# nannau/DoWnGAN

Measured on AMD Instinct MI355X. Metric: train-step samples/sec (G+D+GP), higher is better.
Workload: dtype bf16

## Files before the change

downgan_amd/_lib.py:

```python
from __future__ import annotations

import ctypes as C
import os

_HERE = os.path.dirname(os.path.abspath(__file__))
LIB_PATH = os.environ.get("DG_LIB_OVERRIDE") or os.path.join(_HERE, "csrc", "libdowngan_hip.so")

DG_F32, DG_BF16 = 0, 1
STATUS = {0: "DG_OK", -1: "DG_ERR_BAD_SHAPE", -2: "DG_ERR_BAD_DTYPE", -3: "DG_ERR_BAD_ARG", -4: "DG_ERR_LAUNCH"}


class Epilogue(C.Structure):
    _fields_ = [("bias", C.c_void_p), ("has_act", C.c_int), ("act_slope", C.c_float),
                ("r1", C.c_void_p), ("ldr1", C.c_int64), ("s1", C.c_float),
                ("r2", C.c_void_p), ("ldr2", C.c_int64), ("s2", C.c_float),
                ("mask", C.c_void_p), ("ldmask", C.c_int64), ("mask_slope", C.c_float),
                ("accumulate", C.c_int), ("mask_bits", C.c_void_p), ("out_bits", C.c_void_p),
                ("mask_c0", C.c_int), ("mask_last", C.c_int), ("out_q", C.c_void_p), ("out_qs", C.c_void_p), ("ldqs", C.c_int64),
                ("out_u", C.c_void_p), ("out_ue", C.c_void_p), ("skip_y", C.c_int), ("out_amax", C.c_void_p)]


class ConvGeom(C.Structure):
    _fields_ = [("dtype", C.c_int), ("N", C.c_int), ("H", C.c_int), ("W", C.c_int),
                ("Cin", C.c_int), ("Cout", C.c_int), ("stride", C.c_int), ("cin_real", C.c_int), ("pixel_shuffle", C.c_int),
# ... 83 lines not shown
class Hist2dAxis(C.Structure):
    _fields_ = [("src", C.c_int), ("chan", C.c_int), ("nbins", C.c_int), ("lo", C.c_float), ("inv_w", C.c_float)]


class Hist2dSpec(C.Structure):
    _fields_ = [("npairs", C.c_int), ("speed_u", C.c_int), ("speed_v", C.c_int), ("nsec", C.c_int), ("calm", C.c_float),
                ("tan_k", C.c_float * (HIST2D_MAX_SECTORS // 4)), ("scale", C.c_float * EOF_MAX_C),
                ("offset", C.c_float * EOF_MAX_C), ("ax", (Hist2dAxis * 2) * HIST2D_MAX_PAIRS)]


class IncrSpec(C.Structure):
    _fields_ = [("speed_u", C.c_int), ("speed_v", C.c_int), ("nlag", C.c_int), ("nbins", C.c_int),
                ("lag", C.c_int * INCR_MAX_LAGS), ("scale", C.c_float * EOF_MAX_C), ("offset", C.c_float * EOF_MAX_C),
                ("lo", (C.c_float * INCR_MAX_LAGS) * HIST_MAX_OUT), ("inv_w", (C.c_float * INCR_MAX_LAGS) * HIST_MAX_OUT)]


class ObjectsSpec(C.Structure):
    _fields_ = [("speed_u", C.c_int), ("speed_v", C.c_int), ("nthr", C.c_int), ("connectivity", C.c_int),
                ("inv_quantum", C.c_float), ("scale", C.c_float * EOF_MAX_C), ("offset", C.c_float * EOF_MAX_C),
                ("thr", (C.c_float * OBJ_MAX_THR) * HIST_MAX_OUT)]


class DistmapSpec(C.Structure):
    _fields_ = [("speed_u", C.c_int), ("speed_v", C.c_int), ("nthr", C.c_int), ("nring", C.c_int), ("cutoff", C.c_int),
                ("scale", C.c_float * EOF_MAX_C), ("offset", C.c_float * EOF_MAX_C),
                ("thr", (C.c_float * DIST_MAX_THR) * HIST_MAX_OUT)]


class TemporalSpec(C.Structure):
    _fields_ = [("speed_u", C.c_int), ("speed_v", C.c_int), ("nthr", C.c_int), ("ndur", C.c_int), ("nlag", C.c_int),
                ("nbins", C.c_int), ("below", C.c_int * TEMPORAL_MAX_THR), ("lag", C.c_int * TEMPORAL_MAX_LAGS),
                ("scale", C.c_float * EOF_MAX_C), ("offset", C.c_float * EOF_MAX_C),
                ("thr", (C.c_float * TEMPORAL_MAX_THR) * HIST_MAX_OUT), ("lo", (C.c_float * TEMPORAL_MAX_LAGS) * HIST_MAX_OUT),
                ("inv_w", (C.c_float * TEMPORAL_MAX_LAGS) * HIST_MAX_OUT)]


MINMAX_PARTS = 256
_vp, _i, _i64, _f = C.c_void_p, C.c_int, C.c_int64, C.c_float
_PROTOS = {
    "dg_conv3x3_fwd": [C.POINTER(ConvGeom), C.POINTER(Epilogue), _vp, _vp, _vp, _vp],
    "dg_conv3x3_dgrad": [C.POINTER(ConvGeom), C.POINTER(Epilogue), _vp, _vp, _vp, _vp],
    "dg_conv3x3_wgrad": [C.POINTER(ConvGeom), _vp, _vp, _vp, _vp, _vp],
    "dg_conv3x3_wgrad_dense": [_vp, _i, _vp, _vp, _vp, _vp, _vp],
    "dg_conv3x3_wgrad_f8": [C.POINTER(ConvGeom), _vp, _vp, _vp, _vp, _vp, _vp],
    "dg_exp_from_amax": [_vp, _i, _i, _vp, _vp],
    "dg_conv3x3_wgrad_dense_f8": [C.POINTER(ConvGeom), _i, _vp, _vp, _vp, _vp, _vp, _vp],
    "dg_gather_gemm": [C.POINTER(GGDesc), C.POINTER(Epilogue), _vp, _vp, _vp, _vp],
    "dg_conv3x3_plan": [C.POINTER(ConvGeom), _i, C.POINTER(GGDesc)],
    "dg_last_conv_kernels": [],
    "dg_last_wgrad_kernel": [],
    "dg_conv3x3_dgrad_launches": [C.POINTER(ConvGeom)],
    "dg_conv3x3_dgrad_stream_eligible": [C.POINTER(ConvGeom), C.POINTER(Epilogue)],
    "dg_set_s2_dgrad_stream": [C.c_int],
    "dg_colsum": [_i, _vp, _i64, _i64, _i64, _i64, _i, _vp, _vp],
    "dg_colsum_multi": [_i, _vp, _i64, _i64, _i, _i, _vp, _vp],
    "dg_repack_conv_weights": [_i, _i, _vp, _vp, _i, _i, _vp],
    "dg_repack_dense_dgrad": [_i, _vp, _i, _i, _vp, _vp],
    "dg_wgrad_unswap": [_vp, _vp, _i, _i, _vp],
    "dg_linear_fwd": [_i, _vp, _i64, _vp, _i64, _vp, _i, _i, _i, _i64, _vp],
    "dg_linear_dx": [_i, _i, _vp, _i, _vp, _i64, _vp, _i64, _vp, _i64, _f, _i, _i, _i64, _vp],
    "dg_linear_dw": [_i, _vp, _i, _vp, _i64, _vp, _i64, _i, _i, _i64, _vp],
    "dg_linear_dw_wide": [_i, _vp, _i, _vp, _i64, _vp, _i64, _i, _i, _i64, _i, _vp],
    "dg_bias_act": [_i, _vp, _i, _vp, _vp, _i, _i, _i, _i, _f, _vp, _i, _f, _vp],
    "dg_mask_mul": [_i, _vp, _i64, _vp, _i64, _i64, _i, _f, _vp],
    "dg_axpby": [_i, _vp, _i64, _vp, _i64, _f, _vp, _i64, _f, _i64, _i, _vp],
    "dg_gp_interp": [_i, _vp, _vp, _vp, _vp, _i, _i64, _vp],
    "dg_gp_interp_c2": [_i, _vp, _vp, _i64, _vp, _vp, _vp, _vp, _i, _i64, _vp],
    "dg_scale_rows_c2": [_i, _vp, _i64, _vp, _vp, _i, _i64, _vp],
    "dg_sumsq_rows": [_i, _vp, _i, _i64, _vp, _vp],
    "dg_gp_finish": [_vp, _i, _i, _f, _f, _vp, _vp, _vp],
    "dg_scale_rows": [_i, _vp, _vp, _vp, _i, _i64, _vp],
    "dg_l1": [_i, _vp, _i64, _vp, _i64, _i64, _i, _vp, _vp, _i64, _f, _vp, _i64, _vp],
    "dg_sqdiff": [_i, _vp, _i64, _vp, _i64, _i64, _i, _vp, _vp],
    "dg_sum_strided": [_vp, _i, _i, _f, _vp, _vp],
    "dg_fill_col": [_vp, _i, _i, _i, _f, _vp],
    "dg_adam": [_vp, _vp, _vp, _vp, _vp, _i64, _f, _f, _f, _f, _i, _f, _vp],
    "dg_nchw_to_nhwc": [_i, _vp, _vp, _i, _i, _i, _i, _i, _vp],
    "dg_nhwc_to_nchw": [_i, _vp, _i64, _vp, _i, _i, _i, _i, _vp],
    "dg_cast": [_i, _vp, _vp, _i64, _vp],
    "dg_minmax_partial": [_i, _vp, _i64, _i64, _i, _vp, _vp],
    "dg_minmax_finish": [_vp, _i, _vp, _vp],
    "dg_normalise_planar": [_i, _vp, _i, _i, _i, _i64, _i, _vp, _vp, _vp],
    "dg_ssim_level": [_vp, _vp, _i, _i, _i, C.POINTER(SsimParams), _vp, _vp],
    "dg_avgpool2": [_vp, _vp, _i, _i, _i, _vp],
    "dg_msssim_finish": [_vp, _i, _i, C.POINTER(MsssimCombine), _vp, _vp],
    "dg_div_vort_sums": [_i, _vp, _i64, _vp, _i64, _i, _i, _i, _vp, _vp],
    "dg_gather_samples": [_i, _vp, _i64, _i, _vp, _i, _vp, _i, _vp],
    "dg_quant_mxfp8": [_i, _vp, _i64, _i64, _i, _vp, _i64, _vp, _i64, _vp],
    "dg_block_exp_max": [_vp, _i64, _i64, _i, _i, _vp, _vp, _vp],
    "dg_block_exp_max_batch": [C.POINTER(ExpBatch), _i, _vp, _vp],
    "dg_quant_uniform": [_i, _vp, _i64, _i64, _i, _vp, _vp, _i64, _vp],
    "dg_conv3x3_fwd_f8": [C.POINTER(ConvGeom), C.POINTER(Epilogue), C.POINTER(F8Operands), _vp, _vp],
    "dg_conv3x3_dgrad_f8": [C.POINTER(ConvGeom), C.POINTER(Epilogue), C.POINTER(F8Operands), _vp, _vp],
    "dg_moments": [_vp, _i64, _vp, _vp],
    "dg_stage_fields": [_i, C.POINTER(FieldPlanes), _i64, _vp, _vp],
    "dg_lowpass5": [_i, _vp, _i64, _i, _i, _i, _i, _vp, _i64, _vp, _i64, _vp],
    "dg_lowpass5_adjoint": [_i, _vp, _i64, _i, _i, _i, _i, _vp, _i64, _vp],
    "dg_set_deterministic_workspace": [_vp, _i64],
    "dg_deterministic": [],
    "dg_count_nonfinite": [C.POINTER(FiniteBufs), _vp, _vp],
    "dg_eof_mean": [C.POINTER(EofFields), _vp, _vp],
    "dg_eof_gram": [C.POINTER(EofFields), _vp, _i, _vp, _vp, _vp],
    "dg_eof_components": [C.POINTER(EofFields), _vp, _vp, _i, _vp, _i64, _i64, _vp, _vp],
    "dg_eof_flip": [_vp, _i, _i, _i, _i64, _i64, _vp, _vp],
    "dg_eof_project": [C.POINTER(EofFields), _vp, _vp, _i, _i64, _i64, _i, _vp, _vp, _vp],
    "dg_eof_reconstruct": [_vp, _i, _i, _i, _vp, _i64, _i64, _i, _vp, _vp, _vp],
# ... 107 lines not shown
```

downgan_amd/engine.py:

```python
from __future__ import annotations

import dataclasses
import math
import os

import torch

from . import layout
from .ops import Conv

G_SLOPE = 0.01
C_SLOPE = 0.2
RES_SCALE = 0.2
FC_HID = 100
FC_HID_P = 112
FC_HID_LD = 128
FC_OUT_P = 16


@dataclasses.dataclass
class HyperParams:
    gp_lambda: float = 10.0
    critic_iterations: int = 5
    batch_size: int = 32
# ... 776 lines not shown
            if f8b:
                o.quant_mxfp8(bw["us"][(3 * i + 2) & 1][..., 4 * F_:], *usq((3 * i + 2) & 1, 4 * F_, 5 * F_))
                if u_live:
                    o.quant_uniform(bw["us"][(3 * i + 2) & 1][..., 4 * F_:], *uu(3 * i + 2, 4 * F_, 5 * F_))
            for j in (2, 1, 0):
                d = 3 * i + j
                slab, us = self._saved[d], bw["us"][d & 1]
                pre = f"res_blocks.{i}.dense_blocks.{j}.b"
                for k in range(4, 0, -1):
                    uk = us[..., (k - 1) * F_:k * F_]
                    kw = dict(xq=usq(d & 1, k * F_, 5 * F_), wq=self._vq[d][k], out_q=usq(d & 1, (k - 1) * F_, k * F_)) if f8b else {}
                    if u_live:
                        kw["out_u"] = uu(d, (k - 1) * F_, k * F_)
                    o.conv_dgrad(self.cv_v[k], us[..., k * F_:], self.vpack(d, k), uk, mask=slab[..., k * F_:(k + 1) * F_], mask_slope=G_SLOPE, **kw)
                if u_live:
                    o.conv_wgrad_dense_f8(self.cv_b, self._slab_u[d], self._ex[d], self._us_u[d & 1], self._eu[d], [GW(f"{pre}{k}.0") for k in range(1, 6)])
                    o.colsum_multi(us, [GB(f"{pre}{k}.0") for k in range(1, 6)])
                else:
                    o.conv_wgrad_dense(self.cv_b, slab, us, [GW(f"{pre}{k}.0") for k in range(1, 6)], [GB(f"{pre}{k}.0") for k in range(1, 6)])
                if self.f8_wg:
                    o.block_exp_max(bw["usq"][d & 1][1], self._eu_new[d])
                nxt = bw["us"][(d - 1) & 1][..., 4 * F_:] if j > 0 else bw["gx"]
                kw = {}
                if f8b:
                    kw = dict(xq=usq(d & 1, 0, 5 * F_), wq=self._vq[d][0])
                    if j > 0:
                        kw["out_q"] = usq((d - 1) & 1, 4 * F_, 5 * F_)
                        if u_live:
                            kw["out_u"] = uu(d - 1, 4 * F_, 5 * F_)
                o.conv_dgrad(self.cv_v[0], us, self.vpack(d, 0), nxt, r1=us[..., 4 * F_:], s1=RES_SCALE, **kw)
            gyn = bw["gy"][gyi ^ 1]
            o.axpby(gyn, bw["gx"], 1.0 / RES_SCALE, gy, 1.0)
            gy, gyi = gyn, gyi ^ 1
        if self.f8_wg and self._ex_new is not None:
            self._ex.copy_(self._ex_new); self._eu.copy_(self._eu_new)
            self._u_ok = True
            self._u_live = False
        o.axpby(gy, gy, 1.0, d_trunk, 1.0)
        o.conv_wgrad(self.cv_conv1, x, gy, GW("conv1"), db=GB("conv1"))


METRIC_SINKS = (("spectra", True), ("coherence", False), ("helmholtz", False), ("distributions", True), ("maps", False),
                ("fss", False), ("joint", False), ("increments", False), ("hist_maps", False), ("temporal", False),
                ("objects", False), ("distances", False))


class TrainEngine:

    SCALARS = ("c_real_mean", "c_fake_mean", "gp_ret", "g_c_fake_mean", "l1_sum")

    def __init__(self, ops, coarse_side, filters, channels, batch, hp: HyperParams = None, n_predictands=2,
                 num_res_blocks=16, num_upsample=3, dist=None, stacked=None, check_finite=False):
        self.ops, self.hp = ops, hp or HyperParams()
        self.check_finite = bool(check_finite)
        self.B, self.S = batch, coarse_side
        self.dist = dist
        self.world = dist.world_size if dist is not None else 1
        fine = coarse_side << num_upsample
        self.G = NativeGenerator(ops, filters, channels, batch, coarse_side, n_predictands, num_res_blocks, num_upsample)
        compact2 = n_predictands <= 2 and fine % 32 == 0 and not any(
            os.environ.get(k) is not None for k in ("DG_NO_COMPACT2", "DG_WG_NOIM2COL", "DG_GG_NOIM2COL"))
        if stacked is None:
            env = os.environ.get("DG_STACKED")
            stacked = (int(env) if env.isdigit() and int(env) > 1 else True) if env is not None else False
        stacked = stacked if (stacked and compact2 and self._fits_stacked(ops, filters, batch, coarse_side, fine, num_res_blocks)) else False
        self.C = NativeCritic(ops, filters, fine, n_predictands, batch, stacked=stacked)
        assert self.C.c_pad[0] == self.G.np_p
        o = ops
        self.fine_shape = (batch, fine, fine, self.G.np_p)
        self.compact2 = compact2 and bool(self.C.convs[0].cin_real)
        self.stacked = self.C.stacked and self.compact2
        cshape = (batch, fine, fine, 2) if self.compact2 else self.fine_shape
        self.gbuf = o.zeros(*self.fine_shape)
        self.vbuf = o.zeros(*cshape)
        if self.compact2:
            self.x3 = o.zeros(3 * batch, fine, fine, 2)
            self.real_c, self.fake_c, self.xhat = self.x3[:batch], self.x3[batch:2 * batch], self.x3[2 * batch:]
        else:
            self.x3 = self.real_c = self.fake_c = None
            self.xhat = o.zeros(*cshape)
        self.dfake = None
        self.ss = o.zeros(batch, dtype=torch.float32)
        self.coef = o.zeros(batch, dtype=torch.float32)
        self.scal = o.zeros(8, dtype=torch.float32)
        self.alpha_dev = o.zeros(batch, dtype=torch.float32)
        self.num_steps = 0
        self.n_real_elems = batch * n_predictands * fine * fine
        self.adam_hp = {}
        self._msssim = {}
        self.graphs = False

    def _sc(self, name):
        i = self.SCALARS.index(name)
        return self.scal[i:i + 1]

    @staticmethod
    def _fits_stacked(ops, filters, batch, coarse_side, fine, nrb):
        if not torch.cuda.is_available() or getattr(ops, "device", None) is None or torch.device(ops.device).type != "cuda":
            return True
        es = 4 if ops.tdtype == torch.float32 else 2
        cd, h, per_c = filters, fine, 0
        for l, st in enumerate(NativeCritic.STRIDES):
            h //= st
            per_c += (cd << (l // 2)) * h * h
        critic = 2 * 3 * batch * per_c * es * 1.07 + 2 * batch * cd * fine * fine * es + 24 * (cd * 8 * (fine // 16) ** 2 * 112 + 5e7 * (cd / 128.0) ** 2)
        S, F_ = coarse_side, filters
# ... 251 lines not shown
```

downgan_amd/ops.py:

```python
from __future__ import annotations

import ctypes as C
import dataclasses

import os
import torch

from . import _lib
from ._lib import ConvGeom, Epilogue, check

TORCH_DTYPE = {"f32": torch.float32, "bf16": torch.bfloat16}
DG_DTYPE = {"f32": _lib.DG_F32, "bf16": _lib.DG_BF16}


@dataclasses.dataclass(frozen=True)
class Conv:
    N: int
    H: int
    W: int
    Cin: int
    Cout: int
    stride: int = 1
    pixel_shuffle: bool = False
    cin_real: int = 0
# ... 16 lines not shown

def pix_layout(t):
    assert t.dim() == 4 and t.stride(3) == 1, (t.shape, t.stride())
    ld = t.stride(2)
    n, h, w, _ = t.shape
    assert (w == 1 or t.stride(2) == ld) and (h == 1 or t.stride(1) == w * ld) and (n == 1 or t.stride(0) == h * w * ld), \
        (t.shape, t.stride())
    return ld, n * h * w


_DET = {"ws": None, "refs": 0}


def _det_acquire(lib, device, nbytes):
    if _DET["ws"] is None or _DET["ws"].numel() < nbytes or _DET["ws"].device != torch.device(device):
        ws = torch.empty(nbytes, dtype=torch.uint8, device=device)
        torch.cuda.synchronize(device)
        check(lib.dg_set_deterministic_workspace(C.c_void_p(ws.data_ptr()), ws.numel()), "dg_set_deterministic_workspace")
        _DET["ws"] = ws
    _DET["refs"] += 1


def _det_release(lib):
    _DET["refs"] = max(0, _DET["refs"] - 1)
    if _DET["refs"] == 0 and _DET["ws"] is not None:
        lib.dg_set_deterministic_workspace(C.c_void_p(0), 0)
        _DET["ws"] = None


class HipOps:

    name = "hip"

    def __init__(self, dtype="bf16", device="cuda:0", f8_critic=False, f8_generator=False, deterministic=None, det_workspace_mb=512):
        assert dtype in TORCH_DTYPE
        if not torch.cuda.is_available():
            raise RuntimeError("downgan_amd.ops.HipOps needs a ROCm GPU (no CPU fallback exists)")
        self.dtype = dtype
        self.tdtype = TORCH_DTYPE[dtype]
        self.dg = DG_DTYPE[dtype]
        self.device = torch.device(device)
        self._dev_index = self.device.index if self.device.index is not None else torch.cuda.current_device()
        self.lib = _lib.lib()
        self.prof = None
        self.f8 = bool(f8_critic or f8_generator)
        self.f8_generator = bool(f8_generator)
        self.f8_wgrad = os.environ.get("DG_NO_F8_WGRAD") is None
        self.f8_gbwd = os.environ.get("DG_NO_F8_GBWD") is None
        self.f8_gwgrad = os.environ.get("DG_NO_F8_GWGRAD") is None
        self.f8_gtail = os.environ.get("DG_NO_F8_GTAIL") is None
        self.f8_l0u = os.environ.get("DG_NO_F8_L0U") is None
        assert not self.f8 or dtype == "bf16", "the fp8 conv path quantises bf16 tensors"
        self._f8_scratch = {}
        if deterministic is None:
            deterministic = os.environ.get("DG_DETERMINISTIC", "0") not in ("", "0")
        self._det_held = False
        if deterministic:
            _det_acquire(self.lib, self.device, int(det_workspace_mb) << 20)
            self._det_held = True
        self._finite_counts = None

    @property
    def deterministic(self):
        return bool(self.lib.dg_deterministic())

    def close(self):
        if self._det_held:
            self._det_held = False
            _det_release(self.lib)

    def __del__(self):
        try:
            self.close()
        except Exception:
            pass

    def count_nonfinite(self, bufs):
        assert 1 <= len(bufs) <= _lib.FINITE_MAX
        f = _lib.FiniteBufs(nbuf=len(bufs))
        for i, (name, t) in enumerate(bufs):
            assert t.is_cuda and t.is_contiguous() and t.dtype in (torch.float32, torch.bfloat16), (name, t.dtype)
            f.ptr[i], f.n[i], f.dtype[i] = t.data_ptr(), t.numel(), (_lib.DG_F32 if t.dtype == torch.float32 else _lib.DG_BF16)
        if self._finite_counts is None:
            self._finite_counts = torch.zeros(_lib.FINITE_MAX, dtype=torch.int32, device=self.device)
        check(self.lib.dg_count_nonfinite(C.byref(f), _ptr(self._finite_counts), self._stream()), "dg_count_nonfinite")
        counts = self._finite_counts.cpu().tolist()
        return {name: int(counts[i]) for i, (name, _) in enumerate(bufs)}

    def _stream(self):
        if torch.cuda.current_device() != self._dev_index:
            torch.cuda.set_device(self.device)
        return C.c_void_p(torch.cuda.current_stream(self.device).cuda_stream)

    per_layer = False

    def _timed(self, tag, flops, fn, nbytes=0.0, net="", geom=""):
        if self.prof is None:
            return fn()
        s, e = torch.cuda.Event(enable_timing=True), torch.cuda.Event(enable_timing=True)
        s.record()
        rc = fn()
        e.record()
        if self.per_layer and geom:
            tag = f"{tag}:{geom}"
        if net:
            tag = f"{tag}:{net}"
# ... 60 lines not shown
        ep.accumulate = int(accumulate)
        for name, t in (("mask_bits", mask_bits), ("out_bits", out_bits)):
            if t is not None:
                assert t.dtype == torch.int16 and t.is_cuda and t.is_contiguous() and tuple(t.shape) == self.bits_shape(out.shape), (name, t.shape, out.shape)
                setattr(ep, name, t.data_ptr())
        assert not (mask is not None and mask_bits is not None)
        if out_q is not None:
            q, qs = out_q
            Cc = out.shape[-1]
            assert out.dtype == torch.bfloat16 and Cc % 64 == 0 and Cc >= 128
            assert q.dtype == torch.uint8 and qs.dtype == torch.uint8 and q.shape == out.shape and q.stride() == out.stride(), (q.shape, q.stride(), out.stride())
            assert tuple(qs.shape) == tuple(out.shape[:-1]) + (Cc // 32,) and qs.stride(-1) == 1
            assert all(qs.stride(i) * out.stride(2) == out.stride(i) * qs.stride(2) for i in range(3)), (qs.stride(), out.stride())
            ep.out_q, ep.out_qs, ep.ldqs = q.data_ptr(), qs.data_ptr(), qs.stride(2)
        if out_u is not None:
            u, ue = out_u
            assert u.dtype == torch.uint8 and u.shape == out.shape and u.stride() == out.stride()
            assert ue.dtype == torch.uint8 and ue.is_contiguous() and ue.numel() == out.shape[-1] // 32
            ep.out_u, ep.out_ue = u.data_ptr(), ue.data_ptr()
        if skip_y:
            assert (out_q is not None or out_u is not None) and not accumulate
            ep.skip_y = 1
        if out_amax is not None:
            assert out_amax.dtype == torch.int32 and out_amax.is_cuda and out_amax.is_contiguous() and out_amax.numel() == out.shape[-1] // 32
            ep.out_amax = out_amax.data_ptr()
        return ep

    def out_shape(self, cv: Conv):
        if cv.pixel_shuffle:
            return (cv.N, 2 * cv.Ho, 2 * cv.Wo, cv.Cout // 4)
        return (cv.N, cv.Ho, cv.Wo, cv.Cout)

    def f8_eligible(self, cv: Conv, kind):
        if kind == "wgrad":
            return (self.f8 and self.f8_wgrad and cv.net == "C" and not cv.pixel_shuffle and cv.Cin % 128 == 0
                    and cv.Cout % 128 == 0 and cv.Wo % 64 == 0)
        cred, nout = (cv.Cin, cv.Cout) if kind == "fwd" else (cv.Cout, cv.Cin)
        nets = ("C", "G") if (self.f8_generator and (kind == "fwd" or self.f8_gbwd)) else ("C",)
        if self.f8_generator and self.f8_gtail and kind == "fwd" and cv.net == "T":
            return cred % 128 == 0 and nout > 64 and (not cv.pixel_shuffle or (cv.Cout // 4) % 32 == 0)
        return self.f8 and cv.net in nets and cred % 128 == 0 and nout > 64 and not cv.pixel_shuffle

    def conv_fwd(self, cv: Conv, x, w_fwd, y, xq=None, wq=None, **ep):
        self._act(x); self._act(y); self._act(w_fwd)
        assert tuple(x.shape) == (cv.N, cv.H, cv.W, cv.Cin) or (cv.cin_real and tuple(x.shape) == (cv.N, cv.H, cv.W, 2) and cv.stride == 1), (x.shape, cv)
        assert tuple(y.shape) == self.out_shape(cv), (y.shape, cv)
        assert w_fwd.numel() == cv.Cout * 9 * cv.Cin and w_fwd.is_contiguous()
        g = self._geom(cv, pix_layout(x)[0], pix_layout(y)[0])
        e = self._epilogue(y, **ep)
        if self.f8_eligible(cv, "fwd"):
            check(self._timed("conv_fwd", self.conv_flops(cv), lambda: self._conv_f8(self.lib.dg_conv3x3_fwd_f8, g, e, x, w_fwd, cv.Cout, cv.Cin, y, xq, wq),
                              self.conv_bytes(cv, ep), cv.net, self._geom_tag(cv)), "dg_conv3x3_fwd_f8")
            return
        check(self._timed("conv_fwd", self.conv_flops(cv), lambda: self.lib.dg_conv3x3_fwd(
            C.byref(g), C.byref(e), _ptr(x), _ptr(w_fwd), _ptr(y), self._stream()), self.conv_bytes(cv, ep), cv.net, self._geom_tag(cv)), "dg_conv3x3_fwd")

    def conv_dgrad(self, cv: Conv, dy, w_dgrad, dx, xq=None, wq=None, **ep):
        self._act(dy); self._act(dx); self._act(w_dgrad)
        assert tuple(dx.shape) == (cv.N, cv.H, cv.W, cv.Cin), (dx.shape, cv)
        assert tuple(dy.shape) == self.out_shape(cv), (dy.shape, cv)
        assert w_dgrad.numel() == cv.Cout * 9 * cv.Cin and w_dgrad.is_contiguous()
        g = self._geom(cv, pix_layout(dx)[0], pix_layout(dy)[0])
        e = self._epilogue(dx, **ep)
        if self.f8_eligible(cv, "dgrad"):
            check(self._timed("conv_dgrad", self.conv_flops(cv), lambda: self._conv_f8(self.lib.dg_conv3x3_dgrad_f8, g, e, dy, w_dgrad, cv.Cin, cv.Cout, dx, xq, wq),
                              self.conv_bytes(cv, ep), cv.net, self._geom_tag(cv)), "dg_conv3x3_dgrad_f8")
            return
        check(self._timed("conv_dgrad", self.conv_flops(cv), lambda: self.lib.dg_conv3x3_dgrad(
            C.byref(g), C.byref(e), _ptr(dy), _ptr(w_dgrad), _ptr(dx), self._stream()), self.conv_bytes(cv, ep), cv.net, self._geom_tag(cv)), "dg_conv3x3_dgrad")

    def quant_mxfp8(self, src, q=None, scales=None):
        Cc = src.shape[-1]
        assert Cc % 128 == 0 and src.stride(-1) == 1 and src.is_cuda and src.dtype in (torch.float32, torch.bfloat16)
        if src.dim() == 4:
            ld, rows = pix_layout(src)
        else:
            assert src.dim() == 2
            ld, rows = src.stride(0), src.shape[0]
        if q is None:
            q = torch.empty(src.shape, dtype=torch.uint8, device=self.device)
            scales = torch.empty(tuple(src.shape[:-1]) + (Cc // 32,), dtype=torch.uint8, device=self.device)
        assert q.dtype == torch.uint8 and scales.dtype == torch.uint8 and q.shape == src.shape and q.stride(-1) == 1 and scales.stride(-1) == 1
        assert tuple(scales.shape) == tuple(src.shape[:-1]) + (Cc // 32,)
        ldq, ldqs = q.stride(-2), scales.stride(-2)
        if src.dim() == 4:
            assert pix_layout(q)[1] == rows and all(scales.stride(i) * ldq == q.stride(i) * ldqs for i in range(3))
        sdt = _lib.DG_F32 if src.dtype == torch.float32 else _lib.DG_BF16
        check(self.lib.dg_quant_mxfp8(sdt, _ptr(src), rows, ld, Cc, _ptr(q), ldq, _ptr(scales), ldqs, self._stream()), "dg_quant_mxfp8")
        return q, scales

    def block_exp_max(self, scales, out, margin=1):
        self.block_exp_max_batch([(scales, out)], margin)

    def block_exp_max_batch(self, pairs, margin=1):
        if self._exp_scratch is None:
            self._exp_scratch = torch.zeros(64 * _lib.EXP_BATCH_MAX, dtype=torch.int32, device=self.device)
        for k in range(0, len(pairs), _lib.EXP_BATCH_MAX):
            b = _lib.ExpBatch()
            chunk = pairs[k:k + _lib.EXP_BATCH_MAX]
            b.n = len(chunk)
            nbytes = 0
            for i, (scales, out) in enumerate(chunk):
                nb = scales.shape[-1]
                assert scales.dtype == torch.uint8 and out.dtype == torch.uint8 and out.numel() == nb and scales.stride(-1) == 1
                assert scales.dim() == 2 or all(scales.stride(d) == scales.stride(d + 1) * scales.shape[d + 1] for d in range(scales.dim() - 2)), scales.stride()
                b.scales[i], b.rows[i], b.ld[i], b.nblocks[i], b.out[i] = scales.data_ptr(), scales.numel() // nb, scales.stride(-2), nb, out.data_ptr()
                nbytes += scales.numel()
# ... 713 lines not shown
```

include/downgan_hip.h:

```cpp
#ifndef DOWNGAN_HIP_H
#define DOWNGAN_HIP_H

#include <stddef.h>
#include <stdint.h>

#ifdef __cplusplus
extern "C" {
#endif

#define DG_F32 0
#define DG_BF16 1

typedef enum dg_status {
  DG_OK = 0,
  DG_ERR_BAD_SHAPE = -1,
  DG_ERR_BAD_DTYPE = -2,
  DG_ERR_BAD_ARG = -3,
  DG_ERR_LAUNCH = -4
} dg_status;

typedef struct dg_epilogue {
  const float* bias;
  int has_act;
  float act_slope;
// ... 27 lines not shown

typedef struct dg_gg_desc {
  int dtype;
  int N, Hs, Ws, Cred; int64_t lds;
  int src_ps;
  int Hg, Wg, sy_mul, sx_mul;
  int ntaps; int tap_dy[9], tap_dx[9], tap_w[9];
  int Nout; int64_t ldw;
  int Hd, Wd; int64_t ldd;
  int dy_mul, dx_mul, dy_off, dx_off;
  int dst_ps;
} dg_gg_desc;

const char* dg_version(void);


int dg_conv3x3_fwd(const dg_conv_geom* g, const dg_epilogue* ep, const void* x, const void* w_fwd,
                   void* y, void* stream);

int dg_conv3x3_dgrad(const dg_conv_geom* g, const dg_epilogue* ep, const void* dy,
                     const void* w_dgrad, void* dx, void* stream);

int dg_conv3x3_wgrad(const dg_conv_geom* g, const void* x, const void* dy, float* dw, float* db,
                     void* stream);

int dg_conv3x3_wgrad_dense(const dg_conv_geom* g, int nconv, const void* x, const void* dy,
                           float* const* dw, float* const* db, void* stream);

int dg_conv3x3_wgrad_f8(const dg_conv_geom* g, const void* xq, const void* ex, const void* dyq, const void* ey, float* dw,
                        void* stream);

int dg_conv3x3_wgrad_dense_f8(const dg_conv_geom* g, int nconv, const void* xq, const void* ex, const void* dyq, const void* ey,
                              float* const* dw, void* stream);

int dg_colsum(int dtype, const void* dy, int64_t rows_outer, int64_t ld_outer, int64_t rows_inner,
              int64_t ld, int C, float* db, void* stream);

int dg_colsum_multi(int dtype, const void* dy, int64_t rows, int64_t ld, int C, int nseg, float* const* db, void* stream);

int dg_gather_gemm(const dg_gg_desc* d, const dg_epilogue* ep, const void* x, const void* w, void* y,
                   void* stream);

int dg_last_conv_kernels(void);

int dg_last_wgrad_kernel(void);

int dg_conv3x3_plan(const dg_conv_geom* g, int kind, dg_gg_desc* out);

int dg_conv3x3_dgrad_launches(const dg_conv_geom* g);

int dg_conv3x3_dgrad_stream_eligible(const dg_conv_geom* g, const dg_epilogue* ep);

int dg_set_s2_dgrad_stream(int on);

int dg_repack_conv_weights(int dtype, int kind, const float* master, void* dst, int CoutP, int CinP,
                           void* stream);
int dg_repack_dense_dgrad(int dtype, const float* const* masters, int nconv, int F, void* dst, void* stream);
int dg_wgrad_unswap(const float* tmp, float* dw, int CoutP, int CinP, void* stream);


int dg_linear_fwd(int dtype, const void* x, int64_t ldx, const void* w, int64_t ldw, float* y,
                  int ldy, int B, int O, int64_t K, void* stream);
int dg_linear_dx(int dtype, int out_dtype, const float* dy, int ldo, const void* w, int64_t ldw,
                 void* dx, int64_t lddx, const void* mask, int64_t ldmask, float mask_slope, int B,
                 int O, int64_t K, void* stream);
int dg_linear_dw(int dtype, const float* dy, int ldo, const void* x, int64_t ldx, float* dw,
                 int64_t lddw, int B, int O, int64_t K, void* stream);
int dg_linear_dw_wide(int dtype, const float* dy, int ldo, const void* x, int64_t ldx, float* dw,
                      int64_t lddw, int B, int O, int64_t K, int accumulate, void* stream);


int dg_bias_act(int out_dtype, const float* in, int ldi, const float* bias, void* out, int ldo,
                int rows, int C, int has_act, float slope, const void* mask, int ldmask,
                float mask_slope, void* stream);
int dg_mask_mul(int dtype, void* u, int64_t ldu, const void* y, int64_t ldy, int64_t rows, int C,
                float slope, void* stream);
int dg_axpby(int dtype, void* out, int64_t ldo, const void* x, int64_t ldx, float a, const void* y,
             int64_t ldy, float b, int64_t rows, int C, void* stream);
int dg_gp_interp(int dtype, const void* real, const void* fake, const float* alpha, void* xhat,
                 int B, int64_t per_img, void* stream);
int dg_gp_interp_c2(int dtype, const void* real, const void* fake, int64_t ld, const float* alpha,
                    void* xhat_c, void* real_c, void* fake_c, int B, int64_t pix_per_img, void* stream);
int dg_scale_rows_c2(int dtype, const void* g, int64_t ld, const float* coef, void* out_c, int B,
                     int64_t pix_per_img, void* stream);
int dg_sumsq_rows(int dtype, const void* g, int B, int64_t per_img, float* ss, void* stream);
int dg_gp_finish(const float* ss, int B, int B_global, float gp_lambda, float weight, float* coef,
                 float* scalars, void* stream);
int dg_scale_rows(int dtype, const void* g, const float* coef, void* out, int B, int64_t per_img,
                  void* stream);
int dg_l1(int dtype, const void* a, int64_t lda, const void* b, int64_t ldb, int64_t rows, int C,
          float* acc, void* grad, int64_t ldg, float grad_scale, const void* addend, int64_t ldadd,
          void* stream);
int dg_sqdiff(int dtype, const void* a, int64_t lda, const void* b, int64_t ldb, int64_t rows, int C,
              float* acc, void* stream);
int dg_sum_strided(const float* in, int n, int stride, float scale, float* out, void* stream);
int dg_fill_col(float* buf, int rows, int ld, int col, float value, void* stream);

int dg_adam(float* p, const float* g, float* m, float* v, void* shadow_bf16, int64_t n, float lr,
            float beta1, float beta2, float eps, int step, float grad_scale, void* stream);

int dg_nchw_to_nhwc(int dtype, const float* src, void* dst, int N, int C, int H, int W, int Cpad,
                    void* stream);
int dg_nhwc_to_nchw(int dtype, const void* src, int64_t lds, float* dst, int N, int C, int H, int W,
                    void* stream);
int dg_cast(int dtype, const float* src, void* dst, int64_t n, void* stream);

// ... 263 lines not shown
```

Baseline: 73.89.

## Add persistent row-streaming 3x3 conv forward kernel with split-K wave handoff

Adds a persistent bf16 3x3 conv forward kernel for Cin=128 stride-1 layers. Each block walks column strips of an image row by row, keeps an 8-row input ring in LDS, and holds weights in registers. Two wave groups each compute half of the input channels and pass partial accumulators through LDS, while the next rows are prefetched with buffer loads. The engine turns this path on by default and falls back to the old kernel for geometries or epilogues it cannot handle. The aim is to cut repeated halo/input loads and launch overhead, at the cost of high register pressure and one block per CU.

```diff
diff --git a/downgan_amd/_lib.py b/downgan_amd/_lib.py
--- a/downgan_amd/_lib.py
+++ b/downgan_amd/_lib.py
@@ -159,6 +159,9 @@
     "dg_conv3x3_dgrad_launches": [C.POINTER(ConvGeom)],
     "dg_conv3x3_dgrad_stream_eligible": [C.POINTER(ConvGeom), C.POINTER(Epilogue)],
     "dg_set_s2_dgrad_stream": [C.c_int],
+    "dg_conv3x3_fwd_stream": [C.POINTER(ConvGeom), C.POINTER(Epilogue), _vp, _vp, _vp, _vp],
+    "dg_conv3x3_fwd_stream_eligible": [C.POINTER(ConvGeom), C.POINTER(Epilogue)],
+    "dg_set_fwd_stream": [C.c_int],
     "dg_colsum": [_i, _vp, _i64, _i64, _i64, _i64, _i, _vp, _vp],
     "dg_colsum_multi": [_i, _vp, _i64, _i64, _i, _i, _vp, _vp],
     "dg_repack_conv_weights": [_i, _i, _vp, _vp, _i, _i, _vp],
diff --git a/downgan_amd/csrc/conv_fwd_stream.hip b/downgan_amd/csrc/conv_fwd_stream.hip
--- /dev/null
+++ b/downgan_amd/csrc/conv_fwd_stream.hip
@@ -0,0 +1,322 @@
+#include "gg_common.h"
+
+namespace {
+
+constexpr int NT = 512;
+constexpr int RING_PIX = 18;
+constexpr int RING_PITCH = 288;
+constexpr int RING_ROW = RING_PIX * RING_PITCH;
+constexpr int RING_SLOTS = 8;
+constexpr int ROW_CHUNKS = RING_PIX * 16;
+constexpr int HAND_OFF = RING_SLOTS * RING_ROW;
+constexpr int HAND_WAVE = 4 * 64 * 16;
+constexpr int HAND_BUF = 4 * HAND_WAVE;
+constexpr int LDS_BYTES = HAND_OFF + 2 * HAND_BUF;
+
+struct FSArgs {
+  const char* x; const char* w; char* y;
+  const float* bias; const char* mask_bits; char* out_bits;
+  float act_slope, mask_slope;
+  int H, W, ldx, ldy;
+  int bpp;
+  int nct;
+  int nstrips, nitems;
+  int nwalk, trips;
+  int xcd_group;
+};
+
+__device__ __forceinline__ __amdgpu_buffer_rsrc_t uniform_rsrc(const char* p) {
+  const unsigned long long b = (unsigned long long)p;
+  const unsigned long long u = ((unsigned long long)(unsigned)__builtin_amdgcn_readfirstlane((int)(unsigned)(b >> 32)) << 32) |
+                               (unsigned)__builtin_amdgcn_readfirstlane((int)(unsigned)b);
+  return __builtin_amdgcn_make_buffer_rsrc((void*)u, 0, (int)DG_OOB_OFF, 0x00020000);
+}
+
+template <int F>
+__device__ __forceinline__ void store_pixel(const FSArgs& a, const f32x4_t& f0, const f32x4_t& f1, unsigned mb, __amdgpu_buffer_rsrc_t rY,
+                                            unsigned off, __amdgpu_buffer_rsrc_t rB, unsigned boff) {
+  float v[8] = {f0[0], f0[1], f0[2], f0[3], f1[0], f1[1], f1[2], f1[3]};
+  if (F & 1) {
+    if (a.act_slope >= 0.f && a.act_slope <= 1.f) {
+      typedef float f32x2_t __attribute__((ext_vector_type(2)));
+      const f32x2_t sl2 = {a.act_slope, a.act_slope};
+#pragma unroll
+      for (int k = 0; k < 8; k += 2) {
+        const f32x2_t p = f32x2_t{v[k], v[k + 1]} * sl2;
+        v[k] = __builtin_fmaxf(v[k], p[0]); v[k + 1] = __builtin_fmaxf(v[k + 1], p[1]);
+      }
+    } else {
+#pragma unroll
+      for (int k = 0; k < 8; ++k) v[k] = leaky(v[k], a.act_slope);
+    }
+  }
+  if (F & 2) {
+#pragma unroll
+    for (int e = 0; e < 8; ++e) v[e] *= ((mb >> e) & 1u) ? 1.f : a.mask_slope;
+  }
+  u32x4_t t;
+#pragma unroll
+  for (int k = 0; k < 4; ++k) t[k] = pack_bf16x2(v[2 * k], v[2 * k + 1]);
+  __builtin_amdgcn_raw_buffer_store_b128(t, rY, off, 0, 0);
+  if (F & 4) {
+    unsigned ob = 0;
+#pragma unroll
+    for (int e = 0; e < 8; ++e) ob |= (v[e] > 0.f ? 1u : 0u) << e;
+    __builtin_amdgcn_raw_buffer_store_b8((unsigned char)ob, rB, boff, 0, 0);
+  }
+}
+
+template <int F, bool KA>
+__device__ __forceinline__ void fs_run(const FSArgs& a, char* lds) {
+  constexpr int CB = KA ? 0 : 1;
+  const int tid = threadIdx.x, lane = tid & 63, q = (tid >> 6) & 3;
+  const int l15 = lane & 15, g = lane >> 4;
+  const int wave = __builtin_amdgcn_readfirstlane(tid >> 6);
+
+  int ct, wlk;
+  if (a.xcd_group) {
+    const int slot = (int)blockIdx.x >> 3;
+    ct = slot % a.nct; wlk = (slot / a.nct) * 8 + ((int)blockIdx.x & 7);
+  } else {
+    ct = (int)blockIdx.x % a.nct; wlk = (int)blockIdx.x / a.nct;
+  }
+
+  uint4 wr[36];
+#pragma unroll
+  for (int t = 0; t < 9; ++t)
+#pragma unroll
+    for (int kk = 0; kk < 2; ++kk)
+#pragma unroll
+      for (int j = 0; j < 2; ++j) {
+        const int n = ct * 128 + 32 * q + 8 * (l15 >> 2) + 4 * j + (l15 & 3);
+        wr[(t * 2 + kk) * 2 + j] = *reinterpret_cast<const uint4*>(a.w + ((long long)n * 1152 + t * 128 + 64 * CB + 32 * kk + 8 * g) * 2);
+      }
+  f32x4_t bias[2] = {f32x4_t{0.f, 0.f, 0.f, 0.f}, f32x4_t{0.f, 0.f, 0.f, 0.f}};
+  if (KA && a.bias) {
+#pragma unroll
+    for (int j = 0; j < 2; ++j) {
+      const float4 b4 = *reinterpret_cast<const float4*>(a.bias + ct * 128 + 32 * q + 8 * g + 4 * j);
+      bias[j] = f32x4_t{b4.x, b4.y, b4.z, b4.w};
+    }
+  }
+
+  const char* const fb0 = lds + l15 * RING_PITCH + g * 16 + CB * 128;
+  char* const hand = lds + HAND_OFF + q * HAND_WAVE + lane * 16;
+  int f_row[3], f_dst[3], f_pix[3];
+#pragma unroll
+  for (int i = 0; i < 3; ++i) {
+    const int ci = tid + 256 * i;
+    f_row[i] = ci >= ROW_CHUNKS ? 1 : 0;
+    const int c = ci - f_row[i] * ROW_CHUNKS;
+    f_pix[i] = c >> 4;
+    f_dst[i] = f_pix[i] * RING_PITCH + (c & 15) * 16;
+  }
+  const bool fill3 = wave == 0;
+  const unsigned rowstep = (unsigned)a.W * (unsigned)a.ldx * 2u;
+  const int nsteps = (a.H + 1) >> 1;
+
+  for (int trip = 0; trip < a.trips; ++trip) {
+    const int item = wlk + trip * a.nwalk;
+    if (item >= a.nitems) break;
+    const int img = item / a.nstrips, x0 = (item - img * a.nstrips) * 16;
+    const __amdgpu_buffer_rsrc_t rX = uniform_rsrc(a.x + (long long)img * a.H * a.W * a.ldx * 2);
+    const __amdgpu_buffer_rsrc_t rY = uniform_rsrc(a.y + (long long)img * a.H * a.W * a.ldy * 2 + ct * 256);
+    const char* const bits = (F & 2) ? a.mask_bits : (F & 4) ? a.out_bits : a.y;
+    const __amdgpu_buffer_rsrc_t rB = uniform_rsrc(bits + (long long)img * a.H * a.W * a.bpp + ct * 16);
+    unsigned f_off[3];
+#pragma unroll
+    for (int i = 0; i < 3; ++i) {
+      const int col = x0 - 1 + f_pix[i];
+      f_off[i] = (KA && (i < 2 || fill3) && (unsigned)col < (unsigned)a.W) ? (unsigned)col * (unsigned)a.ldx * 2u + (unsigned)(tid & 15) * 16u : DG_OOB_OFF;
+    }
+    auto fetch = [&](int r0, u32x4_t (&r)[3]) {
+#pragma unroll
+      for (int i = 0; i < 3; ++i) {
+        if (i == 2 && !fill3) break;
+        const int rr = r0 + f_row[i];
+        r[i] = __builtin_amdgcn_raw_buffer_load_b128(rX, (unsigned)rr < (unsigned)a.H ? f_off[i] + (unsigned)rr * rowstep : DG_OOB_OFF, 0, 0);
+      }
+    };
+    auto put = [&](int r0, const u32x4_t (&r)[3]) {
+#pragma unroll
+      for (int i = 0; i < 3; ++i) {
+        if (i == 2 && !fill3) break;
+        *reinterpret_cast<uint4*>(lds + ((r0 + f_row[i]) & 7) * RING_ROW + f_dst[i]) = __builtin_bit_cast(uint4, r[i]);
+      }
+    };
+    const unsigned pix_ok = x0 + l15 < a.W ? 0u : DG_OOB_OFF;
+    const unsigned st_lane = pix_ok | ((unsigned)(x0 + l15) * (unsigned)a.ldy * 2u + (unsigned)(64 * q + 16 * g));
+    const unsigned bt_lane = pix_ok | ((unsigned)(x0 + l15) * (unsigned)a.bpp + (unsigned)(4 * q + g));
+    const unsigned ystep = (unsigned)a.W * (unsigned)a.ldy * 2u, bstep = (unsigned)a.W * (unsigned)a.bpp;
+
+    u32x4_t st0[3], st1[3];
+    if (KA) {
+      fetch(-1, st0); fetch(1, st1);
+      put(-1, st0); put(1, st1);
+      fetch(3, st0);
+    }
+    __syncthreads();
+
+    auto step = [&](int k, const u32x4_t (&staged)[3], u32x4_t (&nxt)[3]) __attribute__((always_inline)) {
+      const int s = KA ? k : k - 1;
+      const bool on = KA ? k < nsteps : k >= 1;
+      if (on) {
+        f32x4_t acc[2][2];
+        unsigned mb[2] = {0u, 0u};
+        if constexpr (KA) {
+          fetch(2 * k + 5, nxt);
+#pragma unroll
+          for (int rr = 0; rr < 2; ++rr)
+#pragma unroll
+            for (int j = 0; j < 2; ++j) acc[rr][j] = bias[j];
+        } else {
+          if (F & 2) {
+#pragma unroll
+            for (int rr = 0; rr < 2; ++rr)
+              mb[rr] = __builtin_amdgcn_raw_buffer_load_b8(rB, 2 * s + rr < a.H ? bt_lane + (unsigned)(2 * s + rr) * bstep : DG_OOB_OFF, 0, 0);
+          }
+#pragma unroll
+          for (int rr = 0; rr < 2; ++rr)
+#pragma unroll
+            for (int j = 0; j < 2; ++j) acc[rr][j] = *reinterpret_cast<const f32x4_t*>(hand + (s & 1) * HAND_BUF + (rr * 2 + j) * 1024);
+        }
+        auto finish_row = [&](int rr) __attribute__((always_inline)) {
+          if constexpr (KA) {
+#pragma unroll
+            for (int j = 0; j < 2; ++j) *reinterpret_cast<f32x4_t*>(hand + (s & 1) * HAND_BUF + (rr * 2 + j) * 1024) = acc[rr][j];
+          } else {
+            const unsigned rok = 2 * s + rr < a.H ? 0u : DG_OOB_OFF;
+            store_pixel<F>(a, acc[rr][0], acc[rr][1], mb[rr], rY, rok | (st_lane + (unsigned)(2 * s + rr) * ystep), rB,
+                           rok | (bt_lane + (unsigned)(2 * s + rr) * bstep));
+          }
+        };
+        uint4 fb[2][2];
+        auto read_group = [&](int n, uint4 (&b)[2]) __attribute__((always_inline)) {
+          const int i = n / 3, sx = n - 3 * i;
+          const char* const p = fb0 + ((2 * s - 1 + i) & 7) * RING_ROW + sx * RING_PITCH;
+          b[0] = *reinterpret_cast<const uint4*>(p);
+          b[1] = *reinterpret_cast<const uint4*>(p + 64);
+        };
+        read_group(0, fb[0]);
+#pragma unroll
+        for (int n = 0; n < 12; ++n) {
+          const int i = n / 3, sx = n - 3 * i;
+          if (n + 1 < 12) read_group(n + 1, fb[(n + 1) & 1]);
+          __builtin_amdgcn_sched_barrier(0);
+#pragma unroll
+          for (int kk = 0; kk < 2; ++kk) {
+            if (i <= 2) {
+#pragma unroll
+              for (int j = 0; j < 2; ++j) Mma<bf16_t>::run(wr[((i * 3 + sx) * 2 + kk) * 2 + j], fb[n & 1][kk], acc[0][j]);
+            }
+            if (i >= 1) {
+#pragma unroll
+              for (int j = 0; j < 2; ++j) Mma<bf16_t>::run(wr[(((i - 1) * 3 + sx) * 2 + kk) * 2 + j], fb[n & 1][kk], acc[1][j]);
+            }
+          }
+          if (n == 9) finish_row(0);
+          __builtin_amdgcn_sched_barrier(0);
+        }
+        finish_row(1);
+        if constexpr (KA) put(2 * k + 3, staged);
+      }
+      __syncthreads();
+    };
+    for (int k = 0; k <= nsteps; k += 2) {
+      step(k, st0, st1);
+      if (k + 1 <= nsteps) step(k + 1, st1, st0);
+    }
+  }
+}
+
+std::atomic<int> g_fwd_stream{1};
+std::atomic<int> g_cus{0};
+
+}
+
+template <int F>
+__global__ __launch_bounds__(NT, 1) void conv_fwd_stream_kernel(const FSArgs a) {
+  extern __shared__ __attribute__((aligned(16))) char fs_lds[];
+  if (__builtin_amdgcn_readfirstlane(threadIdx.x >> 6) < 4) fs_run<F, true>(a, fs_lds);
+  else fs_run<F, false>(a, fs_lds);
+}
+
+static bool fwd_stream_eligible(const dg_conv_geom* g, const dg_epilogue* ep) {
+  if (!g || g->dtype != DG_BF16 || g->stride != 1 || g->pixel_shuffle || g->cin_real != 0) return false;
+  if (g->N <= 0 || g->H < 8 || g->W < 8) return false;
+  if (g->Cin != 128 || g->ldx < 128 || g->ldx % 8) return false;
+  if (g->Cout < 128 || g->Cout % 128 || g->ldy < g->Cout || g->ldy % 8) return false;
+  if (!gg_halo_row_step_ok(g->W, g->ldx, g->dtype, 1)) return false;
+  if ((long long)g->H * g->W * g->ldx * 2 >= (1ll << 31) || (long long)g->H * g->W * g->ldy * 2 >= (1ll << 31)) return false;
+  if (ep) {
+    if (ep->r1 || ep->r2 || ep->mask || ep->accumulate || ep->mask_c0 || ep->mask_last || ep->out_q || ep->out_qs || ep->out_u || ep->out_ue ||
+        ep->skip_y || ep->out_amax)
+      return false;
+    if (ep->mask_bits && (ep->bias || ep->has_act || ep->out_bits)) return false;
+  }
+  return true;
+}
+
+template <int F>
+static int fwd_stream_launch_f(const FSArgs& a, int grid, hipStream_t st) {
+  DG_SET_MAX_LDS_ONCE((&conv_fwd_stream_kernel<F>), LDS_BYTES);
+  hipLaunchKernelGGL(conv_fwd_stream_kernel<F>, dim3(grid), dim3(NT), LDS_BYTES, st, a);
+  return dg_check_launch();
+}
+
+static int fwd_stream_launch(const dg_conv_geom* g, const dg_epilogue* ep, const void* x, const void* w, void* y, int mode, hipStream_t st) {
+  if (!x || !w || !y) return DG_ERR_BAD_ARG;
+  int cus = g_cus.load(std::memory_order_relaxed);
+  if (cus <= 0) {
+    int dev = 0;
+    if (hipGetDevice(&dev) != hipSuccess || hipDeviceGetAttribute(&cus, hipDeviceAttributeMultiprocessorCount, dev) != hipSuccess || cus <= 0)
+      return DG_ERR_LAUNCH;
+    g_cus.store(cus, std::memory_order_relaxed);
+  }
+  FSArgs a{};
+  a.x = (const char*)x; a.w = (const char*)w; a.y = (char*)y;
+  a.act_slope = 1.f; a.mask_slope = 1.f;
+  int F = 0;
+  if (ep) {
+    a.bias = ep->bias; a.mask_bits = (const char*)ep->mask_bits; a.out_bits = (char*)ep->out_bits;
+    a.act_slope = ep->act_slope; a.mask_slope = ep->mask_slope;
+    F = (ep->has_act ? 1 : 0) | (ep->mask_bits ? 2 : 0) | (ep->out_bits ? 4 : 0);
+  }
+  a.H = g->H; a.W = g->W; a.ldx = (int)g->ldx; a.ldy = (int)g->ldy;
+  a.bpp = g->Cout / 8; a.nct = g->Cout / 128;
+  a.nstrips = (g->W + 15) / 16;
+  const long long items = (long long)g->N * a.nstrips;
+  if (items >= (1ll << 31)) return DG_ERR_BAD_SHAPE;
+  a.nitems = (int)items;
+  const int cap = mode > 1 && mode < cus ? mode : cus;
+  a.nwalk = cap / a.nct > 0 ? cap / a.nct : 1;
+  if (a.nwalk > a.nitems) a.nwalk = a.nitems;
+  a.trips = (a.nitems + a.nwalk - 1) / a.nwalk;
+  a.xcd_group = a.nwalk % 8 == 0 ? 1 : 0;
+  const int grid = a.nwalk * a.nct;
+  g_last_kinds |= 128;
+  switch (F) {
+    case 0: return fwd_stream_launch_f<0>(a, grid, st);
+    case 1: return fwd_stream_launch_f<1>(a, grid, st);
+    case 2: return fwd_stream_launch_f<2>(a, grid, st);
+    case 4: return fwd_stream_launch_f<4>(a, grid, st);
+    case 5: return fwd_stream_launch_f<5>(a, grid, st);
+    default: return DG_ERR_BAD_ARG;
+  }
+}
+
+extern "C" int dg_set_fwd_stream(int n) { return g_fwd_stream.exchange(n < 0 ? 0 : n, std::memory_order_relaxed); }
+
+extern "C" int dg_conv3x3_fwd_stream_eligible(const dg_conv_geom* g, const dg_epilogue* ep) {
+  dg_gg_desc d[4];
+  const int n = dg_conv3x3_plan(g, 0, d);
+  if (n < 0) return n;
+  return fwd_stream_eligible(g, ep) ? 1 : 0;
+}
+
+extern "C" int dg_conv3x3_fwd_stream(const dg_conv_geom* g, const dg_epilogue* ep, const void* x, const void* w_fwd, void* y, void* stream) {
+  const int mode = g_fwd_stream.load(std::memory_order_relaxed);
+  if (!mode || dg_conv3x3_fwd_stream_eligible(g, ep) != 1) return dg_conv3x3_fwd(g, ep, x, w_fwd, y, stream);
+  g_last_kinds = 0;
+  return fwd_stream_launch(g, ep, x, w_fwd, y, mode, reinterpret_cast<hipStream_t>(stream));
+}
diff --git a/downgan_amd/engine.py b/downgan_amd/engine.py
--- a/downgan_amd/engine.py
+++ b/downgan_amd/engine.py
@@ -852,6 +852,8 @@
     def __init__(self, ops, coarse_side, filters, channels, batch, hp: HyperParams = None, n_predictands=2,
                  num_res_blocks=16, num_upsample=3, dist=None, stacked=None, check_finite=False):
         self.ops, self.hp = ops, hp or HyperParams()
+        if hasattr(ops, "stream_fwd") and os.environ.get("DG_FWD_STREAM") != "0":
+            ops.stream_fwd = True
         self.check_finite = bool(check_finite)
         self.B, self.S = batch, coarse_side
         self.dist = dist
diff --git a/downgan_amd/ops.py b/downgan_amd/ops.py
--- a/downgan_amd/ops.py
+++ b/downgan_amd/ops.py
@@ -92,6 +92,7 @@
         self.f8_l0u = os.environ.get("DG_NO_F8_L0U") is None
         assert not self.f8 or dtype == "bf16", "the fp8 conv path quantises bf16 tensors"
         self._f8_scratch = {}
+        self.stream_fwd = False
         if deterministic is None:
             deterministic = os.environ.get("DG_DETERMINISTIC", "0") not in ("", "0")
         self._det_held = False
@@ -258,7 +259,8 @@
             check(self._timed("conv_fwd", self.conv_flops(cv), lambda: self._conv_f8(self.lib.dg_conv3x3_fwd_f8, g, e, x, w_fwd, cv.Cout, cv.Cin, y, xq, wq),
                               self.conv_bytes(cv, ep), cv.net, self._geom_tag(cv)), "dg_conv3x3_fwd_f8")
             return
-        check(self._timed("conv_fwd", self.conv_flops(cv), lambda: self.lib.dg_conv3x3_fwd(
+        fwd = self.lib.dg_conv3x3_fwd_stream if self.stream_fwd else self.lib.dg_conv3x3_fwd
+        check(self._timed("conv_fwd", self.conv_flops(cv), lambda: fwd(
             C.byref(g), C.byref(e), _ptr(x), _ptr(w_fwd), _ptr(y), self._stream()), self.conv_bytes(cv, ep), cv.net, self._geom_tag(cv)), "dg_conv3x3_fwd")
 
     def conv_dgrad(self, cv: Conv, dy, w_dgrad, dx, xq=None, wq=None, **ep):
diff --git a/include/downgan_hip.h b/include/downgan_hip.h
--- a/include/downgan_hip.h
+++ b/include/downgan_hip.h
@@ -103,6 +103,12 @@
 int dg_conv3x3_dgrad_stream_eligible(const dg_conv_geom* g, const dg_epilogue* ep);
 
 int dg_set_s2_dgrad_stream(int on);
+
+int dg_conv3x3_fwd_stream(const dg_conv_geom* g, const dg_epilogue* ep, const void* x, const void* w_fwd, void* y, void* stream);
+
+int dg_conv3x3_fwd_stream_eligible(const dg_conv_geom* g, const dg_epilogue* ep);
+
+int dg_set_fwd_stream(int n);
 
 int dg_repack_conv_weights(int dtype, int kind, const float* master, void* dst, int CoutP, int CinP,
                            void* stream);
```

Result: no change. 74.37 (median of 6 runs) (+0.6%).
